# BaratiLab/GAMD

Measured on AMD Instinct MI355X. Metric: atom-steps/sec (force eval + integrate), 10k-atom LJ box, higher is better.
Workload: dtype f32; 1 GPU; C2: 10 000-atom LJ box, rho*=0.5, L=92.29 A, cutoff 3.0 sigma=10.2 A, fp32, 4 conv layers x 128, random-init weights (seed 0), 1 box per GPU; n_atoms=10000, boxes=1, launch=single process

## Files before the change

gamd_amd/csrc/conv_edge.hip:

```cpp
#include "gamd_common.h"
#include "gamd_internal.h"

#include <cstdlib>

namespace {

constexpr int conv_lds_floats(bool l0, bool fold = false) { return 2 * GAMD_WFRAG_FLOATS + 3 * 128 + (fold ? 256 : 0); }

template <bool F2, typename Post, typename Mid, typename Tail>
__device__ __forceinline__ void gemm128_post(const f32x4* W, int lane, const f32x16 (&X)[4], f32x16 (&acc)[4], Post post, Mid mid, Tail tail) {
#pragma unroll
    for (int tp = 0; tp < 4; ++tp) {
        if (tp == 1) mid();
#pragma unroll
        for (int t = 0; t < 4; ++t) {
#pragma unroll
            for (int q = 0; q < 4; ++q) {
                const f32x4 w = W[((tp * 4 + t) * 4 + q) * 64 + lane];
#pragma unroll
                for (int j = 0; j < 4; ++j) {
                    const float x = X[t][q * 4 + j];
                    acc[tp] = F2 ? mfma32(x, w[j], acc[tp]) : mfma32(w[j], x, acc[tp]);
                }
                if (tp > 0) post(tp - 1, t * 4 + q);
            }
        }
        tail(tp);
    }
#pragma unroll
    for (int g = 0; g < 16; ++g) post(3, g);
}
template <bool F2, typename Post, typename Mid>
__device__ __forceinline__ void gemm128_post(const f32x4* W, int lane, const f32x16 (&X)[4], f32x16 (&acc)[4], Post post, Mid mid) {
    gemm128_post<F2>(W, lane, X, acc, post, mid, [](int) {});
}

template <int N>
__device__ __forceinline__ void phase_barrier() {
    asm volatile("s_waitcnt vmcnt(%0) lgkmcnt(0)" ::"n"(N) : "memory");
    __builtin_amdgcn_s_barrier();
}

__device__ __forceinline__ void load_e_tile(const float* __restrict__ e_frag, int tile, int lane, f32x16 (&X)[4]) {
    const f32x4* ef = (const f32x4*)e_frag + (size_t)tile * 16 * 64;
#pragma unroll
    for (int t = 0; t < 4; ++t)
#pragma unroll
        for (int q = 0; q < 4; ++q) {
            const f32x4 v = gamd_load_stream(&ef[(t * 4 + q) * 64 + lane]);
#pragma unroll
            for (int j = 0; j < 4; ++j) X[t][q * 4 + j] = v[j];
        }
}

template <bool TIME, bool L0, bool FOLD = false>
__global__ void __launch_bounds__(512, 2) k_conv_edge(ConvEdgeArgs a) {
    if (a.devflags[DEVFLAG_FROZEN]) return;
    extern __shared__ __attribute__((aligned(16))) float lds[];
    float* buf0 = lds + (L0 ? 3 * 128 + (FOLD ? 256 : 0) : 0);
    float* buf1 = buf0 + GAMD_WFRAG_FLOATS;
    float* vb1 = L0 ? lds : buf1 + GAMD_WFRAG_FLOATS;
    float* vb3 = vb1 + 128;
    float* vb4 = vb3 + 128;
    float* vSD0 = vb4;
    float* vax = vb4 + 128;

    const int tid = threadIdx.x, lane = tid & 63, slot = lane & 31, half = lane >> 5;
    const int wave = __builtin_amdgcn_readfirstlane(tid >> 6);
    const unsigned lane16 = (unsigned)lane * 16u;
    int E = a.counters[CNT_E];
    if ((long long)E > a.e_cap) E = (int)a.e_cap;
    const int n_tiles = (E + GAMD_TILE - 1) / GAMD_TILE;
    const int n_units = (n_tiles + 3) / 4;
    int first, end, step;
    gamd_xcd_range(n_units, blockIdx.x, gridDim.x, first, end, step);
    if (first >= end) return;
    const int n_iter = ((end - first + step - 1) / step + 1) / 2;
    const int wsub = wave & 3, whalf = wave >> 2;
    const bool early = whalf == 0;
    auto tile_of = [&](int it) {
        const int u = first + (2 * it + whalf) * step;
        return (it < n_iter && u < end) ? u * 4 + wsub : n_tiles;
    };
    auto stage = [&](const float* gw, float* buf) { gamd_stage_weight_raw_contig<8>(gw, buf, wave, lane16); };

    long long tacc[16];
#pragma unroll
    for (int i = 0; i < 16; ++i) tacc[i] = 0;
    long long tprev = 0;
#define TMARK(i) do { if (TIME) { const long long tn__ = (long long)__builtin_readcyclecounter(); tacc[i] += tn__ - tprev; tprev = tn__; } } while (0)

    float vax_t = 0.f;
    if (FOLD && tid < 256) vax_t = a.w1p[GAMD_WFRAG_FLOATS + tid];
    if (tid < 128) {
        vb1[tid] = a.b1[tid]; vb3[tid] = a.b3[tid];
        if (L0) vSD0[tid] = a.S[tid] + a.D[tid];
        else vb4[tid] = a.b4[tid];
    }
    if (FOLD && tid < 256) vax[tid] = vax_t;
    stage(a.w1p, buf0);

    f32x16 RA[4], RB[4], RC[4];
    float rs = 0.f;
    float wxr[4] = {0.f, 0.f, 0.f, 0.f};
    auto fold_head = [&]() {
        if constexpr (FOLD) {
#pragma unroll
            for (int tp = 0; tp < 4; ++tp) wxr[tp] = vax[tp * 64 + lane];
            asm volatile("" : "+v"(wxr[0]), "+v"(wxr[1]), "+v"(wxr[2]), "+v"(wxr[3]));
        }
    };
    auto fold_tail = [&](int tp) { if constexpr (FOLD) RB[tp] = mfma32(wxr[tp], rs, RB[tp]); };
    auto init_b4 = [&]() {
#pragma unroll
        for (int tp = 0; tp < 4; ++tp) {
            const float b = vb4[32 * tp + slot];
#pragma unroll
            for (int r = 0; r < 16; ++r) RC[tp][r] = b;
        }
    };

    int tile = tile_of(0);
    bool active = tile < n_tiles;
    int src = 0, dst = 0;
    {
        const int x = tile * GAMD_TILE + gamd_pi(slot);
        if (active && x < E) {
            src = GAMD_CHK_RANGE(a.sticky, a.col[x], 0, a.zero_row, GAMD_CHK_CONV_SRC);
            if (!L0) dst = GAMD_CHK_RANGE(a.sticky, a.erow[x], 0, a.zero_row, GAMD_CHK_CONV_DST);
        } else { src = a.zero_row; dst = a.zero_row; }
        if (FOLD && active) rs = a.e_rstd[(size_t)tile * 64 + lane];
        if (active) load_e_tile(a.e_frag, tile, lane, RA);
    }
    asm volatile("" ::"v"(src), "v"(dst));
    asm volatile("s_waitcnt vmcnt(0)" ::: "memory");
    __syncthreads();
    if (TIME) tprev = (long long)__builtin_readcyclecounter();
    unsigned pend_ends = 0;
    int pend_p = 0;

    auto gather_S = [&]() { load_row_chain(a.S + (size_t)src * GAMD_H, half, RA); };
    auto gather_hn = [&]() {
        const unsigned soff = (unsigned)src << 9;
        const unsigned idx0 = 16u * (unsigned)half;
        const unsigned slot16 = 16u * (unsigned)slot;
#pragma unroll
        for (int r4 = 0; r4 < 4; ++r4) {
            unsigned o0, o1, o2, o3;
            asm volatile("ds_bpermute_b32 %0, %4, %5 offset:%6\n\tds_bpermute_b32 %1, %4, %5 offset:%7\n\t"
                         "ds_bpermute_b32 %2, %4, %5 offset:%8\n\tds_bpermute_b32 %3, %4, %5 offset:%9\n\ts_waitcnt lgkmcnt(0)"
                         : "=&v"(o0), "=&v"(o1), "=&v"(o2), "=&v"(o3)
                         : "v"(idx0), "v"(soff), "n"(4 * (0 + 8 * r4)), "n"(4 * (1 + 8 * r4)), "n"(4 * (2 + 8 * r4)), "n"(4 * (3 + 8 * r4)));
            const unsigned o[4] = {o0, o1, o2, o3};
#pragma unroll
            for (int k = 0; k < 4; ++k) {
                const f32x4 hv = *(const f32x4*)((const char*)a.hn + (o[k] + slot16));
#pragma unroll
                for (int tp = 0; tp < 4; ++tp) RA[r4][k * 4 + tp] = hv[tp];
            }
        }
    };

    auto early_barrier = [&](bool gathered) { if (gathered) phase_barrier<16>(); else phase_barrier<0>(); };
    auto early_barrier_e = [&](bool gathered) { if (gathered) phase_barrier<FOLD ? 17 : 16>(); else phase_barrier<0>(); };
    auto piece_stores = [&]() {
        while (__any(pend_ends != 0)) {
            if (pend_ends != 0) {
                const int r = __builtin_ctz(pend_ends);
                pend_ends &= pend_ends - 1;
                f32x4 pv;
#pragma unroll
                for (int tp = 0; tp < 4; ++tp) {
                    float v = RC[tp][0];
#pragma unroll
                    for (int k = 1; k < 16; ++k) v = (r == k) ? RC[tp][k] : v;
                    pv[tp] = v;
                }
                *(f32x4*)(a.partial + (size_t)pend_p * GAMD_H + 4 * slot) = pv;
                ++pend_p;
            }
        }
    };
#define FENCE() __builtin_amdgcn_sched_barrier(0)

    if constexpr (L0) {
    for (int it = 0; it < n_iter; ++it) {
        const int x0 = tile * GAMD_TILE + 16 * half;
        int nvalid = E - x0;
        nvalid = !active ? 0 : (nvalid >= 16 ? 16 : (nvalid <= 0 ? 0 : nvalid));
        const int tile_n = tile_of(it + 1);
// ... 199 lines not shown
```

gamd_amd/csrc/edge_encode.hip:

```cpp
#include "gamd_common.h"
#include "gamd_internal.h"

namespace {

constexpr int ENC_W1_FLOATS = 4 * 6 * 64 * 4;
constexpr int ENC_LDS_FLOATS = ENC_W1_FLOATS + 2 * GAMD_WFRAG_FLOATS + 5 * 128 + 64;
constexpr int ENC_R_FLOATS = 10 * 1024;

__device__ __forceinline__ constexpr int enc_r_block(int tp, int t) { return (tp == 0 ? 0 : tp == 1 ? 4 : tp == 2 ? 7 : 9) + (t - tp); }

template <typename WPtr, typename BPtr>
__device__ __forceinline__ void gemm128_upper_sq(WPtr W, BPtr b, int lane, int half, const f32x16 (&X)[4], float (&vt)[4]) {
#pragma unroll
    for (int tp = 0; tp < 4; ++tp) {
        f32x16 acc;
#pragma unroll
        for (int q = 0; q < 4; ++q) {
            const f32x4 v = *reinterpret_cast<const f32x4*>(&b[32 * tp + 8 * q + 4 * half]);
#pragma unroll
            for (int j = 0; j < 4; ++j) acc[q * 4 + j] = v[j];
        }
#pragma unroll
        for (int t = tp; t < 4; ++t)
#pragma unroll
            for (int q = 0; q < 4; ++q) {
                const f32x4 w = W[(enc_r_block(tp, t) * 4 + q) * 64 + lane];
#pragma unroll
                for (int j = 0; j < 4; ++j) acc = mfma32(w[j], X[t][q * 4 + j], acc);
            }
        vt[tp] = 0.f;
#pragma unroll
        for (int r = 0; r < 16; ++r) vt[tp] = fmaf(acc[r], acc[r], vt[tp]);
    }
}

template <int NFEAT, typename CPtr>
__device__ __forceinline__ void edge_features(const EncArgs& a, CPtr cen, int src, int dst, const float4& ps, const float4& pd,
                                              int half, float (&F)[24]) {
#pragma clang fp contract(off)
    const BoxDims B = gamd_edge_box(a, dst);
    const float rx = gamd_min_image_wrapped(ps.x - pd.x, B.bx, B.hx);
    const float ry = gamd_min_image_wrapped(ps.y - pd.y, B.by, B.hy);
    const float rz = gamd_min_image_wrapped(ps.z - pd.z, B.bz, B.hz);
    const float nrm = sqrtf((rx * rx + ry * ry) + rz * rz);
    const float den = nrm + 1e-8f;
    const float d = (nrm - a.length_mean) / a.length_std;
    F[0] = half ? ry / den : rx / den;
    F[1] = half ? d : rz / den;
    if (a.rbf.uniform) {
        gamd_rbf_chains(d, half, a.gamma * -1.4426950408889634f, a.rbf, F);
    } else {
#pragma unroll
        for (int s = 2; s < 22; ++s) {
            const float radial = d - cen[2 * (s - 2) + half];
            F[s] = __builtin_amdgcn_exp2f((a.gamma * -1.4426950408889634f) * (radial * radial));
        }
    }
    F[22] = 0.f; F[23] = 0.f;
    if (NFEAT == 45) {
        float flag = 0.f;
        if (a.bond_nbr) {
            const int io = a.perm[dst], jo = a.perm[src];
            const int4 nb = *reinterpret_cast<const int4*>(a.bond_nbr + 4 * (size_t)io);
            flag = (nb.x == jo || nb.y == jo || nb.z == jo || nb.w == jo) ? 1.f : 0.f;
        }
        F[22] = half ? 0.f : flag;
    }
}


__device__ __forceinline__ void gelu_block(const f32x16 (&acc)[4], f32x16 (&X)[4], const GeluCoef& k) {
    __builtin_amdgcn_s_setprio(1);
#pragma unroll
    for (int t = 0; t < 4; ++t)
#pragma unroll
        for (int r = 0; r < 16; r += 2) {
            const gelu_f2 y = gelu_pair(gelu_f2{acc[t][r], acc[t][r + 1]}, k);
            X[t][r] = y[0]; X[t][r + 1] = y[1];
        }
    __builtin_amdgcn_s_setprio(0);
}

template <int NFEAT, bool FOLD = false>
__global__ void __launch_bounds__(512, 2) k_edge_encode(EncArgs a) {
    if (a.devflags[DEVFLAG_FROZEN]) return;
    extern __shared__ __attribute__((aligned(16))) float lds[];
    float* w1 = lds;
    float* w2 = w1 + ENC_W1_FLOATS;
    float* w3 = w2 + GAMD_WFRAG_FLOATS;
    float* vb1 = w3 + GAMD_WFRAG_FLOATS;
    float* vb2 = vb1 + 128;
    float* vb3 = vb2 + 128;
    float* vg = vb3 + 128;
    float* vbeta = vg + 128;
    float* cen = vbeta + 128;

    const int tid = threadIdx.x;
    const GeluCoef gk = gelu_coef();
    for (int i = tid; i < ENC_W1_FLOATS / 4; i += 512) ((f32x4*)w1)[i] = ((const f32x4*)a.w1p)[i];
    for (int i = tid; i < GAMD_WFRAG_FLOATS / 4; i += 512) {
        ((f32x4*)w2)[i] = ((const f32x4*)a.w2p)[i];
        if (!FOLD || i < ENC_R_FLOATS / 4) ((f32x4*)w3)[i] = ((const f32x4*)a.w3p)[i];
    }
    if (tid < 128) {
        vb1[tid] = a.b1[tid]; vb2[tid] = a.b2[tid]; vb3[tid] = a.b3[tid];
        if (!FOLD) { vg[tid] = a.ln_g[tid]; vbeta[tid] = a.ln_b[tid]; }
    }
    if (tid < 40) cen[tid] = a.centers[tid];
    __syncthreads();

    const int lane = tid & 63, wave = tid >> 6, slot = lane & 31, half = lane >> 5;
    long long E = a.counters[CNT_E];
    if (E > a.e_cap) E = a.e_cap;
    const int n_tiles = (int)((E + GAMD_TILE - 1) / GAMD_TILE);
    const int n_units = (n_tiles + 3) / 4;
    int first, end, step;
    gamd_xcd_range(n_units, blockIdx.x, gridDim.x, first, end, step);
    const int n_iter = first < end ? ((end - first + step - 1) / step + 1) / 2 : 0;
    auto tile_of = [&](int it) {
        const int u = first + (2 * it + (wave >> 2)) * step;
        return (it < n_iter && u < end) ? u * 4 + (wave & 3) : n_tiles;
    };

    constexpr int KSTEPS = (NFEAT + 1) / 2;

    int E32 = (int)E;
    auto fetch_idx = [&](int tile, int& src, int& dst) -> bool {
        const int x = tile * GAMD_TILE + gamd_pi(slot);
        const bool ok = tile < n_tiles && x < E32;
        const int xc = ok ? x : 0;
        src = GAMD_CHK_RANGE(a.sticky, a.col[xc], 0, a.zero_row, GAMD_CHK_ENC_SRC); dst = GAMD_CHK_RANGE(a.sticky, a.erow[xc], 0, a.zero_row, GAMD_CHK_ENC_DST);
        return ok;
    };
    int src_c, dst_c;
    {
        const bool ok = fetch_idx(tile_of(0), src_c, dst_c);
        src_c = ok ? src_c : 0; dst_c = ok ? dst_c : 0;
    }
    float4 ps = a.pos_s[src_c], pd = a.pos_s[dst_c];

    for (int it = 0; it < n_iter; ++it) {
        const int tile = tile_of(it);
        int src_n, dst_n;
        const bool ok_n = fetch_idx(tile_of(it + 1), src_n, dst_n);
        if (tile >= n_tiles) { asm volatile("" ::"v"(src_n), "v"(dst_n)); continue; }
        const long long x = (long long)tile * GAMD_TILE + gamd_pi(slot);
        const bool valid = x < E;
        const int src = src_c, dst = dst_c;
        float F[24];
        __builtin_amdgcn_s_setprio(1);
        if constexpr (FOLD) edge_features<NFEAT>(a, a.centers, src, dst, ps, pd, half, F);
        else edge_features<NFEAT>(a, cen, src, dst, ps, pd, half, F);
        asm volatile("" : "+v"(F[0]), "+v"(F[23]));
        __builtin_amdgcn_s_setprio(0);
        if (a.feat_dbg && valid) {
#pragma unroll
            for (int s = 0; s < 24; ++s) a.feat_dbg[x * 48 + 2 * s + half] = F[s];
        }

        f32x16 acc[4], X[4];
        load_bias_chain(vb1, half, acc);
#pragma unroll
        for (int tp = 0; tp < 4; ++tp) {
#pragma unroll
            for (int g = 0; g < 6; ++g) {
                if (4 * g >= KSTEPS) break;
                const f32x4 w = ((const f32x4*)w1)[(tp * 6 + g) * 64 + lane];
#pragma unroll
                for (int j = 0; j < 4; ++j)
                    if (4 * g + j < KSTEPS) acc[tp] = mfma32(w[j], F[4 * g + j], acc[tp]);
            }
        }
        gelu_block(acc, X, gk);
        if constexpr (FOLD) {
#pragma unroll
            for (int t = 0; t < 4; ++t) asm volatile("" : "+v"(X[t]));
        }
        load_bias_chain(vb2, half, acc);
        gemm128<false>((const f32x4*)w2, lane, X, acc);
        gelu_block(acc, X, gk);
        src_c = ok_n ? src_n : 0; dst_c = ok_n ? dst_n : 0;
        ps = a.pos_s[src_c]; pd = a.pos_s[dst_c];
        if constexpr (FOLD) {
#pragma unroll
            for (int t = 0; t < 4; ++t) asm volatile("" : "+v"(X[t]));
            float vt[4];
            gemm128_upper_sq((const f32x4*)w3, vb3, lane, half, X, vt);
            const float var = gamd_xhalf_sum((vt[0] + vt[1]) + (vt[2] + vt[3])) * a.ln_inv_width;
            const float rstd = 1.0f / sqrtf(var + 1e-5f);
#pragma unroll
            for (int t = 0; t < 4; ++t)
#pragma unroll
                for (int r = 0; r < 16; ++r) acc[t][r] = X[t][r] * rstd;
// ... 172 lines not shown
```

gamd_amd/csrc/gamd_common.h:

```cpp
#pragma once
#include <hip/hip_runtime.h>
#include <stdint.h>

typedef float f32x16 __attribute__((ext_vector_type(16)));
typedef float f32x4 __attribute__((ext_vector_type(4)));

#define GAMD_H 128
#define GAMD_TILE 32
#define GAMD_CHUNK 16
#define GAMD_WFRAG_FLOATS (GAMD_H * GAMD_H)

__device__ __forceinline__ int gamd_pi(int rho) {
    return 16 * ((rho >> 2) & 1) + (rho & 3) + 4 * (rho >> 3);
}

__device__ __forceinline__ f32x16 mfma32(float a, float b, f32x16 c) {
    return __builtin_amdgcn_mfma_f32_32x32x2f32(a, b, c, 0, 0, 0);
}

template <bool F2, typename WPtr>
__device__ __forceinline__ void gemm128_tile(WPtr W, int lane, const f32x16 (&X)[4], f32x16& acc, int tp) {
#pragma unroll
    for (int t = 0; t < 4; ++t) {
#pragma unroll
// ... 51 lines not shown
    gelu_f2 d;
    asm("v_pk_fma_f32 %0, %1, %2, %3" : "=v"(d) : "v"(a), "v"(b), "v"(c));
    return d;
}
__device__ __forceinline__ gelu_f2 gelu_pair(gelu_f2 x, const GeluCoef& k) {
    const gelu_f2 a = {__builtin_amdgcn_fmed3f(fabsf(x[0]), 0.0f, 6.0f), __builtin_amdgcn_fmed3f(fabsf(x[1]), 0.0f, 6.0f)};
    gelu_f2 q = pk_fma(k.q[6], a, k.q[5]);
    q = pk_fma(q, a, k.q[4]);
    q = pk_fma(q, a, k.q[3]);
    q = pk_fma(q, a, k.q[2]);
    q = pk_fma(q, a, k.q[1]);
    q = pk_fma(q, a, k.q[0]);
    const gelu_f2 e = {__builtin_amdgcn_exp2f(q[0]), __builtin_amdgcn_exp2f(q[1])};
    const gelu_f2 relu = {x[0] - __builtin_amdgcn_fmed3f(x[0], -3.0e38f, 0.0f), x[1] - __builtin_amdgcn_fmed3f(x[1], -3.0e38f, 0.0f)};
    gelu_f2 r = {__builtin_fmaf(-a[0], e[0], relu[0]), __builtin_fmaf(-a[1], e[1], relu[1])};
    return r;
}

struct RbfGrid { int uniform; float c0, delta, A, B, C; };
__device__ __forceinline__ void gamd_rbf_chains(float d, int half, float gexp, const RbfGrid& g, float (&F)[24]) {
#pragma clang fp contract(off)
    const float s = 2.0f * g.delta;
    const float dh = d - (g.c0 + (half ? g.delta : 0.0f));
#pragma unroll
    for (int c = 0; c < 4; ++c) {
        const float u0 = dh - (float)(5 * c) * s;
        float v = __builtin_amdgcn_exp2f(gexp * (u0 * u0));
        float rho = __builtin_amdgcn_exp2f(fmaf(g.A, u0, g.B));
        F[2 + 5 * c] = v;
#pragma unroll
        for (int j = 1; j < 5; ++j) {
            v *= rho;
            F[2 + 5 * c + j] = v;
            if (j < 4) rho *= g.C;
        }
    }
}

__device__ __forceinline__ float gamd_remainder(float a, float b) {
    float m = fmodf(a, b);
    if (m != 0.0f && ((b < 0.0f) != (m < 0.0f))) m += b;
    return m;
}

__device__ __forceinline__ float gamd_min_image_wrapped(float d, float L, float halfL) {
    float t = d + halfL;
    if (t < 0.0f) t += L;
    else if (t >= L) t -= L;
    return t - halfL;
}

__device__ __forceinline__ f32x4 gamd_load_stream(const f32x4* p) { return __builtin_nontemporal_load(p); }

__device__ __forceinline__ float gamd_msg_acc(float hn, float e_emb, float prev) { return __builtin_fmaf(hn, e_emb, prev); }

#define GAMD_L0_PAD (-0x1p100f)
__device__ __forceinline__ float gamd_l0_acc(float pre, float prev) {
    const float e = __builtin_amdgcn_exp2f(pre * -1.4426950408889634f);
    return __builtin_fmaf(pre, __builtin_amdgcn_rcpf(1.0f + e), prev);
}

__host__ __device__ __forceinline__ int gamd_tab16_pos(int f) {
    return 16 * (2 * (f >> 5) + ((f >> 4) & 1)) + 8 * ((f >> 2) & 1) + 4 * ((f >> 3) & 1) + (f & 3);
}

template <typename BPtr>
__device__ __forceinline__ void load_bias_chain(BPtr b, int half, f32x16 (&acc)[4]) {
#pragma unroll
    for (int t = 0; t < 4; ++t)
#pragma unroll
        for (int q = 0; q < 4; ++q) {
            const f32x4 v = *reinterpret_cast<const f32x4*>(&b[32 * t + 8 * q + 4 * half]);
#pragma unroll
            for (int j = 0; j < 4; ++j) acc[t][q * 4 + j] = v[j];
        }
}

__device__ __forceinline__ void load_row_chain(const float* __restrict__ row, int half, f32x16 (&X)[4]) {
#pragma unroll
    for (int t = 0; t < 4; ++t)
#pragma unroll
        for (int q = 0; q < 4; ++q) {
            const f32x4 v = *reinterpret_cast<const f32x4*>(row + 32 * t + 8 * q + 4 * half);
#pragma unroll
            for (int j = 0; j < 4; ++j) X[t][q * 4 + j] = v[j];
        }
}

__device__ __forceinline__ void store_row_chain(float* __restrict__ row, int half, const f32x16 (&X)[4]) {
#pragma unroll
    for (int t = 0; t < 4; ++t)
#pragma unroll
        for (int q = 0; q < 4; ++q) {
            f32x4 v;
#pragma unroll
            for (int j = 0; j < 4; ++j) v[j] = X[t][q * 4 + j];
            *reinterpret_cast<f32x4*>(row + 32 * t + 8 * q + 4 * half) = v;
        }
}

__device__ __forceinline__ float gamd_xhalf_sum(float v) {
    return v + __shfl_xor(v, 32, 64);
}

template <typename GPtr>
__device__ __forceinline__ void layernorm_chain(f32x16 (&X)[4], GPtr gamma, GPtr beta, int half, float eps) {
// ... 20 lines not shown
            const f32x4 g = *reinterpret_cast<const f32x4*>(&gamma[32 * t + 8 * q + 4 * half]);
            const f32x4 b = *reinterpret_cast<const f32x4*>(&beta[32 * t + 8 * q + 4 * half]);
#pragma unroll
            for (int j = 0; j < 4; ++j) X[t][q * 4 + j] = (X[t][q * 4 + j] - mean) * rstd * g[j] + b[j];
        }
}

template <int NW = 8>
__device__ __forceinline__ void gamd_stage_weight(const float* __restrict__ gw, float* ldsbuf, int wave, unsigned lane16) {
    asm volatile("" : "+v"(lane16));
#pragma unroll
    for (int k = 0; k < 64 / NW; ++k) {
        const int chunk = k * NW + wave;
        const char* base = reinterpret_cast<const char*>(gw) + chunk * 1024;
        __builtin_amdgcn_global_load_lds(
            (const __attribute__((address_space(1))) void*)(base + lane16),
            (__attribute__((address_space(3))) void*)(ldsbuf + chunk * 256), 16, 0, 0);
    }
}

#pragma clang diagnostic push
#pragma clang diagnostic ignored "-Winline-asm"

template <int NW = 8>
__device__ __forceinline__ void gamd_stage_weight_raw(const float* __restrict__ gw, float* ldsbuf, int wave, unsigned lane16) {
    const unsigned lds0 = (unsigned)(size_t)(__attribute__((address_space(3))) float*)ldsbuf;
#pragma unroll
    for (int k = 0; k < 64 / NW; ++k) {
        const int chunk = k * NW + wave;
        asm volatile("s_mov_b32 m0, %2\n\ts_nop 0\n\tglobal_load_lds_dwordx4 %0, %1"
                     ::"v"(lane16), "s"(reinterpret_cast<const char*>(gw) + chunk * 1024), "s"(lds0 + chunk * 1024u)
                     : "memory", "m0");
    }
}

template <int NW = 8>
__device__ __forceinline__ void gamd_stage_weight_raw_contig(const float* __restrict__ gw, float* ldsbuf, int wave, unsigned lane16) {
    static_assert((64 / NW) % 4 == 0, "whole groups of four KiB-sized copies per wave");
    int woff = wave * (64 / NW) * 1024;
    asm volatile("" : "+s"(woff));
    const char* g0 = reinterpret_cast<const char*>(gw) + woff;
    const unsigned l0 = (unsigned)(size_t)(__attribute__((address_space(3))) float*)ldsbuf + (unsigned)woff;
#pragma unroll
    for (int h = 0; h < 64 / NW / 4; ++h)
        asm volatile("s_mov_b32 m0, %2\n\ts_nop 0\n\t"
                     "global_load_lds_dwordx4 %0, %1\n\t"
                     "global_load_lds_dwordx4 %0, %1 offset:1024\n\t"
                     "global_load_lds_dwordx4 %0, %1 offset:2048\n\t"
                     "global_load_lds_dwordx4 %0, %1 offset:3072"
                     ::"v"(lane16), "s"(g0 + h * 4096), "s"(l0 + h * 4096u)
                     : "memory", "m0");
}

#pragma clang diagnostic pop

struct WQuarter { f32x4 w[16]; };

__device__ __forceinline__ void load_wquarter(const float* __restrict__ Wp, int quarter, int lane, WQuarter& o) {
    const f32x4* W = reinterpret_cast<const f32x4*>(Wp) + (size_t)quarter * 16 * 64 + lane;
#pragma unroll
    for (int i = 0; i < 16; ++i) o.w[i] = W[i * 64];
}

template <bool F2 = false>
__device__ __forceinline__ void gemm_quarter(const WQuarter& wq, const f32x16 (&X)[4], f32x16& acc) {
#pragma unroll
    for (int t = 0; t < 4; ++t)
#pragma unroll
        for (int q = 0; q < 4; ++q)
#pragma unroll
            for (int j = 0; j < 4; ++j)
                acc = F2 ? mfma32(X[t][q * 4 + j], wq.w[t * 4 + q][j], acc) : mfma32(wq.w[t * 4 + q][j], X[t][q * 4 + j], acc);
}

__device__ __forceinline__ f32x16 load_slice(const float* __restrict__ row, int quarter, int half) {
    f32x16 v;
#pragma unroll
    for (int q = 0; q < 4; ++q) {
        const f32x4 x = *reinterpret_cast<const f32x4*>(row + 32 * quarter + 8 * q + 4 * half);
#pragma unroll
        for (int j = 0; j < 4; ++j) v[q * 4 + j] = x[j];
    }
    return v;
}

__device__ __forceinline__ void store_slice(float* __restrict__ row, int quarter, int half, const f32x16& v) {
#pragma unroll
    for (int q = 0; q < 4; ++q) {
        f32x4 x;
#pragma unroll
        for (int j = 0; j < 4; ++j) x[j] = v[q * 4 + j];
        *reinterpret_cast<f32x4*>(row + 32 * quarter + 8 * q + 4 * half) = x;
    }
}

template <int NB, int XLDW>
__device__ __forceinline__ void exchange_blocks(float* xbuf, int quarter, int slot, int half, const f32x16 (&mine)[NB],
                                                f32x16 (&X)[NB][4]) {
    __syncthreads();
#pragma unroll
    for (int b = 0; b < NB; ++b) store_slice(xbuf + slot * XLDW + 128 * b, quarter, half, mine[b]);
    __syncthreads();
#pragma unroll
    for (int b = 0; b < NB; ++b) load_row_chain(xbuf + slot * XLDW + 128 * b, half, X[b]);
}

// ... 44 lines not shown
```

gamd_amd/csrc/node.hip:

```cpp
#include "gamd_common.h"
#include "gamd_internal.h"

namespace {

typedef _Float16 nf16x8 __attribute__((ext_vector_type(8)));
typedef _Float16 nf16x2 __attribute__((ext_vector_type(2)));
typedef float nf32x2 __attribute__((ext_vector_type(2)));

constexpr int NT = 16;
constexpr int XLD = 136;

__device__ __forceinline__ f32x4 mfma16(float a, float b, f32x4 c) {
    return __builtin_amdgcn_mfma_f32_16x16x4f32(a, b, c, 0, 0, 0);
}

struct WHalf { f32x4 w[8]; };
__device__ __forceinline__ void load_whalf(const float* __restrict__ Wp, int w, int lane, int half, WHalf& h) {
    const f32x4* W = reinterpret_cast<const f32x4*>(Wp) + (size_t)w * 16 * 64 + lane;
#pragma unroll
    for (int o = 0; o < 2; ++o)
#pragma unroll
        for (int b = 0; b < 4; ++b) h.w[o * 4 + b] = W[(o * 8 + 4 * half + b) * 64];
}

// ... 46 lines not shown
    __builtin_amdgcn_sched_barrier(0);
    cur = wn;
    if (NEXT) {
        asm volatile("" ::: "memory");
        load_whalf(next, w, lane, 0, wn);
        asm volatile("" ::: "memory");
    }
    if constexpr (F16) gemm16_half_f16(cur, 1, XB, acc); else gemm16_half(cur, 1, XB, acc);
    __builtin_amdgcn_sched_barrier(0);
}

__device__ __forceinline__ void load16(const float* __restrict__ row, int w, int g, f32x4 (&v)[2]) {
    v[0] = *reinterpret_cast<const f32x4*>(row + 32 * w + 4 * g);
    v[1] = *reinterpret_cast<const f32x4*>(row + 32 * w + 16 + 4 * g);
}
__device__ __forceinline__ void store16(float* __restrict__ row, int w, int g, const f32x4 (&v)[2]) {
    *reinterpret_cast<f32x4*>(row + 32 * w + 4 * g) = v[0];
    *reinterpret_cast<f32x4*>(row + 32 * w + 16 + 4 * g) = v[1];
}

__device__ __forceinline__ void exchange16(float* xbuf, int w, int a, int g, const f32x4 (&mine)[2], f32x4 (&XB)[8]) {
    __syncthreads();
    store16(xbuf + a * XLD, w, g, mine);
    __syncthreads();
#pragma unroll
    for (int blk = 0; blk < 8; ++blk) XB[blk] = *reinterpret_cast<const f32x4*>(xbuf + a * XLD + 16 * blk + 4 * g);
}

typedef _Float16 nf16x4 __attribute__((ext_vector_type(4)));
__device__ __forceinline__ nf16x4 cvt16x4(const f32x4& v) {
    const nf16x2 lo = __builtin_convertvector(nf32x2{v[0], v[1]}, nf16x2), hi = __builtin_convertvector(nf32x2{v[2], v[3]}, nf16x2);
    return nf16x4{lo[0], lo[1], hi[0], hi[1]};
}
__device__ __forceinline__ void store16_h(_Float16* __restrict__ row, int w, int g, const f32x4 (&v)[2]) {
    *reinterpret_cast<nf16x4*>(row + 32 * w + 4 * g) = cvt16x4(v[0]);
    *reinterpret_cast<nf16x4*>(row + 32 * w + 16 + 4 * g) = cvt16x4(v[1]);
}
__device__ __forceinline__ void store16_tab(_Float16* __restrict__ row, int w, int g, const f32x4 (&v)[2]) {
    *reinterpret_cast<nf16x4*>(row + 32 * w + 8 * (g & 1) + 4 * (g >> 1)) = cvt16x4(v[0]);
    *reinterpret_cast<nf16x4*>(row + 32 * w + 16 + 8 * (g & 1) + 4 * (g >> 1)) = cvt16x4(v[1]);
}

__device__ __forceinline__ float group_sum(float v) {
    v += __shfl_xor(v, 16, 64);
    return v + __shfl_xor(v, 32, 64);
}

template <bool F16>
__global__ void __launch_bounds__(256, 3) k_node(NodeArgs a) {
    __shared__ __attribute__((aligned(16))) float xbuf[NT * XLD];
    __shared__ float obuf[4][NT][3];
    __shared__ float red[2][4][NT];

    if (a.counters[CNT_OVERFLOW] || a.devflags[DEVFLAG_FROZEN]) return;
    if (a.mode == 0 && a.l0_gate && a.counters[CNT_REBUILD] == 0) return;

    const int lane = threadIdx.x & 63, la = lane & 15, g = lane >> 4;
    const int w = __builtin_amdgcn_readfirstlane(threadIdx.x >> 6);
    const int atom_raw = blockIdx.x * NT + la;
    const bool valid = atom_raw < a.n;
    const int atom = valid ? atom_raw : a.n - 1;
    const size_t row = (size_t)atom * GAMD_H;

#ifdef GAMD_PROFILING
    long long tm[16] = {0, 0, 0, 0, 0, 0, 0, 0, 0, 0, 0, 0, 0, 0, 0, 0};
#define NMARK(I) do { if (a.tdbg) tm[I] = (long long)__builtin_readcyclecounter(); } while (0)
#else
#define NMARK(I) do { } while (0)
#endif
    NMARK(0);
    f32x4 XB[8];
    XSplit XS;
#define GEMM16(NEXT, W, NXT) do { if constexpr (F16) gemm16<NEXT, true>(W, NXT, wn, XS, mine, w, lane); \
                                  else gemm16<NEXT, false>(W, NXT, wn, XB, mine, w, lane); } while (0)
#define SPLIT16() do { if constexpr (F16) split16(XB, XS); } while (0)
    f32x4 mine[2];
    WHalf wn;

    if (a.mode == 0) {
        if (a.node_emb) {
            load16(a.node_emb, w, g, mine);
        } else {
            const float f = a.pos_s[atom].w;
            f32x4 ww[2];
            load16(a.enc_w, w, g, ww);
            load16(a.enc_b, w, g, mine);
#pragma unroll
            for (int o = 0; o < 2; ++o)
#pragma unroll
                for (int r = 0; r < 4; ++r) mine[o][r] = f * ww[o][r] + mine[o][r];
        }
        if (valid) store16(a.h_out + row, w, g, mine);
        load_whalf(a.pre.wsp, w, lane, 0, wn);
    } else {
        const int rp0 = a.row_ptr[atom], dg = a.deg[atom];
        const int na_incl = a.na_excl[atom] + ((dg > 0 && (rp0 % GAMD_CHUNK) != 0) ? 1 : 0);
        const int p0 = rp0 / GAMD_CHUNK + na_incl;
        const int np = dg > 0 ? ((rp0 + dg - 1) / GAMD_CHUNK - rp0 / GAMD_CHUNK + 1) : 0;
        (void)GAMD_CHK_RANGE(a.sticky, (long long)p0 + np, 0, a.piece_cap, GAMD_CHK_NODE_PIECES);
        float n_real = 0.f;
        if (a.post.c0) {
            float n_pad = 0.f;
            if (a.col) {
#pragma unroll
                for (int k = 0; k < 4; ++k) {
                    const int j = g + 4 * k;
                    if (j < dg && a.col[rp0 + dg - 1 - j] == a.n) n_pad += 1.f;
                }
                n_pad = group_sum(n_pad);
            }
            n_real = (float)dg - n_pad;
        }
        mine[0] = f32x4{0.f, 0.f, 0.f, 0.f};
        mine[1] = mine[0];
        f32x4 p_in[2], h_res[2];
        load16(a.P_in + row, w, g, p_in);
        for (int k0 = 0; __any(k0 < np); k0 += 8) {
            f32x4 pc[8][2];
#pragma unroll
            for (int k = 0; k < 8; ++k) {
                const int kk = (k0 + k < np) ? k0 + k : (np > 0 ? np - 1 : 0);
                load16(a.partial + (size_t)(np > 0 ? p0 + kk : 0) * GAMD_H, w, g, pc[k]);
            }
#pragma unroll
            for (int k = 0; k < 8; ++k)
                if (k0 + k < np) { mine[0] += pc[k][0]; mine[1] += pc[k][1]; }
        }
        NMARK(1);
        asm volatile("" ::: "memory");
        load_whalf(a.post.wpep, w, lane, 0, wn);
        exchange16(xbuf, w, la, g, mine, XB);
        SPLIT16();
        NMARK(2);
        mine[0] = p_in[0]; mine[1] = p_in[1];
        GEMM16(true, a.post.wpep, a.post.wphip);
        if (a.post.c0) {
            f32x4 c[2];
            load16(a.post.c0, w, g, c);
#pragma unroll
            for (int o = 0; o < 2; ++o)
#pragma unroll
                for (int r = 0; r < 4; ++r) mine[o][r] = fmaf(n_real, c[o][r], mine[o][r]);
        }
        NMARK(3);
#pragma unroll
        for (int o = 0; o < 2; ++o)
#pragma unroll
            for (int r = 0; r < 4; ++r) mine[o][r] = gamd_silu_hw(mine[o][r]);
        exchange16(xbuf, w, la, g, mine, XB);
        SPLIT16();
        NMARK(4);
        load16(a.post.bphi, w, g, mine);
        load16(a.h_in + row, w, g, h_res);
        GEMM16(true, a.post.wphip, a.mode != 2 ? a.pre.wsp : a.dec_w1p);
        mine[0] += h_res[0]; mine[1] += h_res[1];
        if (valid) store16(a.h_out + row, w, g, mine);
        NMARK(5);
    }

    if (a.mode != 2) {
        float mean = 0.f, rstd = 1.0f;
        if (!a.norm_bn) {
            float ps = 0.f;
#pragma unroll
            for (int o = 0; o < 2; ++o)
#pragma unroll
                for (int r = 0; r < 4; ++r) ps += mine[o][r];
            ps = group_sum(ps);
            if (g == 0) red[0][w][la] = ps;
// ... 111 lines not shown
```

Before: 3.403 million atom-steps/s.

## Overlap kernel prologue loads with device-flag and edge-count checks

The edge-conv, edge-encode and node kernels now issue the frozen/overflow/edge-count word loads through vector loads and read them later. Edge indices, biases, the first edge tile and the weight staging are issued speculatively before those values arrive, so the prologue memory latency overlaps instead of serialising behind the flag checks. A new tile-map header assigns each block a fixed first unit that needs no edge count, which makes the early speculative index loads possible, and weight staging in edge-encode switches to direct global-to-LDS copies. The cost is wasted speculative loads when the kernel exits early, plus added complexity in the tile scheduling.

```diff
diff --git a/gamd_amd/csrc/conv_edge.hip b/gamd_amd/csrc/conv_edge.hip
--- a/gamd_amd/csrc/conv_edge.hip
+++ b/gamd_amd/csrc/conv_edge.hip
@@ -1,5 +1,6 @@
 #include "gamd_common.h"
 #include "gamd_internal.h"
+#include "gamd_tile_map.h"
 
 #include <cstdlib>
 
@@ -55,7 +56,10 @@
 
 template <bool TIME, bool L0, bool FOLD = false>
 __global__ void __launch_bounds__(512, 2) k_conv_edge(ConvEdgeArgs a) {
-    if (a.devflags[DEVFLAG_FROZEN]) return;
+    const long long t_entry = TIME ? (long long)__builtin_readcyclecounter() : 0;
+    asm volatile("" ::"s"(a.devflags), "s"(a.counters), "s"(a.col), "s"(a.erow), "s"(a.e_frag), "s"(a.e_rstd), "s"(a.e_cap), "s"(a.w1p),
+                 "s"(a.b1), "s"(a.b3), "s"(a.b4), "s"(a.S), "s"(a.D), "s"(gridDim.x));
+    const int frozen_v = gamd_head_word_issue(a.devflags + DEVFLAG_FROZEN), E_v = gamd_head_word_issue(a.counters + CNT_E);
     extern __shared__ __attribute__((aligned(16))) float lds[];
     float* buf0 = lds + (L0 ? 3 * 128 + (FOLD ? 256 : 0) : 0);
     float* buf1 = buf0 + GAMD_WFRAG_FLOATS;
@@ -68,21 +72,41 @@
     const int tid = threadIdx.x, lane = tid & 63, slot = lane & 31, half = lane >> 5;
     const int wave = __builtin_amdgcn_readfirstlane(tid >> 6);
     const unsigned lane16 = (unsigned)lane * 16u;
-    int E = a.counters[CNT_E];
+    const int wsub = wave & 3, whalf = wave >> 2;
+    const bool early = whalf == 0;
+    auto stage = [&](const float* gw, float* buf) { gamd_stage_weight_raw_contig<8>(gw, buf, wave, lane16); };
+
+    f32x16 RA[4], RB[4], RC[4];
+    float rs = 0.f;
+    const int tile0 = gamd_tile_map_unit0(blockIdx.x, gridDim.x, whalf) * 4 + wsub;
+    const bool cap0 = (long long)tile0 * GAMD_TILE < a.e_cap;
+    int src_raw, dst_raw = 0;
+    {
+        const long long x = (long long)tile0 * GAMD_TILE + gamd_pi(slot);
+        const int xc = x < a.e_cap ? (int)x : 0;
+        src_raw = a.col[xc];
+        if (!L0) dst_raw = a.erow[xc];
+    }
+    if (FOLD && cap0 && early) rs = a.e_rstd[(size_t)tile0 * 64 + lane];
+    if (cap0 && early) load_e_tile(a.e_frag, tile0, lane, RA);
+    float vax_t = 0.f, vb1_t = 0.f, vb3_t = 0.f, vb4_t = 0.f, vd0_t = 0.f;
+    if (FOLD && tid < 256) vax_t = a.w1p[GAMD_WFRAG_FLOATS + tid];
+    if (tid < 128) {
+        vb1_t = a.b1[tid]; vb3_t = a.b3[tid];
+        if (L0) { vb4_t = a.S[tid]; vd0_t = a.D[tid]; }
+        else vb4_t = a.b4[tid];
+    }
+    stage(a.w1p, buf0);
+    asm volatile("" ::: "memory");
+    if (gamd_head_word(frozen_v)) { asm volatile("s_waitcnt vmcnt(0)" ::: "memory"); return; }
+    int E = gamd_head_word(E_v);
     if ((long long)E > a.e_cap) E = (int)a.e_cap;
     const int n_tiles = (E + GAMD_TILE - 1) / GAMD_TILE;
     const int n_units = (n_tiles + 3) / 4;
-    int first, end, step;
-    gamd_xcd_range(n_units, blockIdx.x, gridDim.x, first, end, step);
-    if (first >= end) return;
-    const int n_iter = ((end - first + step - 1) / step + 1) / 2;
-    const int wsub = wave & 3, whalf = wave >> 2;
-    const bool early = whalf == 0;
-    auto tile_of = [&](int it) {
-        const int u = first + (2 * it + whalf) * step;
-        return (it < n_iter && u < end) ? u * 4 + wsub : n_tiles;
-    };
-    auto stage = [&](const float* gw, float* buf) { gamd_stage_weight_raw_contig<8>(gw, buf, wave, lane16); };
+    const GamdTileMap tmap = gamd_tile_map(n_units, blockIdx.x, gridDim.x);
+    if (tmap.n_iter == 0) { asm volatile("s_waitcnt vmcnt(0)" ::: "memory"); return; }
+    const int n_iter = tmap.n_iter;
+    auto tile_of = [&](int it) { return gamd_tile_map_tile_later(tmap, it, whalf, wsub, n_tiles); };
 
     long long tacc[16];
 #pragma unroll
@@ -90,18 +114,6 @@
     long long tprev = 0;
 #define TMARK(i) do { if (TIME) { const long long tn__ = (long long)__builtin_readcyclecounter(); tacc[i] += tn__ - tprev; tprev = tn__; } } while (0)
 
-    float vax_t = 0.f;
-    if (FOLD && tid < 256) vax_t = a.w1p[GAMD_WFRAG_FLOATS + tid];
-    if (tid < 128) {
-        vb1[tid] = a.b1[tid]; vb3[tid] = a.b3[tid];
-        if (L0) vSD0[tid] = a.S[tid] + a.D[tid];
-        else vb4[tid] = a.b4[tid];
-    }
-    if (FOLD && tid < 256) vax[tid] = vax_t;
-    stage(a.w1p, buf0);
-
-    f32x16 RA[4], RB[4], RC[4];
-    float rs = 0.f;
     float wxr[4] = {0.f, 0.f, 0.f, 0.f};
     auto fold_head = [&]() {
         if constexpr (FOLD) {
@@ -120,22 +132,30 @@
         }
     };
 
-    int tile = tile_of(0);
+    int tile = gamd_tile_map_tile(tmap, 0, whalf, wsub, n_tiles);
     bool active = tile < n_tiles;
-    int src = 0, dst = 0;
+    int src = a.zero_row, dst = L0 ? 0 : a.zero_row;
     {
         const int x = tile * GAMD_TILE + gamd_pi(slot);
         if (active && x < E) {
-            src = GAMD_CHK_RANGE(a.sticky, a.col[x], 0, a.zero_row, GAMD_CHK_CONV_SRC);
-            if (!L0) dst = GAMD_CHK_RANGE(a.sticky, a.erow[x], 0, a.zero_row, GAMD_CHK_CONV_DST);
-        } else { src = a.zero_row; dst = a.zero_row; }
-        if (FOLD && active) rs = a.e_rstd[(size_t)tile * 64 + lane];
-        if (active) load_e_tile(a.e_frag, tile, lane, RA);
+            src = GAMD_CHK_RANGE(a.sticky, src_raw, 0, a.zero_row, GAMD_CHK_CONV_SRC);
+            if (!L0) dst = GAMD_CHK_RANGE(a.sticky, dst_raw, 0, a.zero_row, GAMD_CHK_CONV_DST);
+        }
     }
     asm volatile("" ::"v"(src), "v"(dst));
+    if (tid < 128) {
+        vb1[tid] = vb1_t; vb3[tid] = vb3_t;
+        if (L0) vSD0[tid] = vb4_t + vd0_t;
+        else vb4[tid] = vb4_t;
+    }
+    if (FOLD && tid < 256) vax[tid] = vax_t;
     asm volatile("s_waitcnt vmcnt(0)" ::: "memory");
     __syncthreads();
-    if (TIME) tprev = (long long)__builtin_readcyclecounter();
+    if (!early && active) {
+        if (FOLD) rs = a.e_rstd[(size_t)tile * 64 + lane];
+        load_e_tile(a.e_frag, tile, lane, RA);
+    }
+    if (TIME) { tprev = (long long)__builtin_readcyclecounter(); tacc[14] = tprev - t_entry; }
     unsigned pend_ends = 0;
     int pend_p = 0;
 
diff --git a/gamd_amd/csrc/edge_encode.hip b/gamd_amd/csrc/edge_encode.hip
--- a/gamd_amd/csrc/edge_encode.hip
+++ b/gamd_amd/csrc/edge_encode.hip
@@ -1,5 +1,6 @@
 #include "gamd_common.h"
 #include "gamd_internal.h"
+#include "gamd_tile_map.h"
 
 namespace {
 
@@ -83,7 +84,24 @@
 
 template <int NFEAT, bool FOLD = false>
 __global__ void __launch_bounds__(512, 2) k_edge_encode(EncArgs a) {
-    if (a.devflags[DEVFLAG_FROZEN]) return;
+    asm volatile("" ::"s"(a.devflags), "s"(a.counters), "s"(a.col), "s"(a.erow), "s"(a.e_cap), "s"(a.pos_s), "s"(a.w1p), "s"(a.w2p), "s"(a.w3p),
+                 "s"(gridDim.x));
+    const int frozen_v = gamd_head_word_issue(a.devflags + DEVFLAG_FROZEN), E_v = gamd_head_word_issue(a.counters + CNT_E);
+    int src_raw, dst_raw;
+    {
+        const int wave0 = __builtin_amdgcn_readfirstlane(threadIdx.x >> 6);
+        const long long x = (long long)(gamd_tile_map_unit0(blockIdx.x, gridDim.x, wave0 >> 2) * 4 + (wave0 & 3)) * GAMD_TILE + gamd_pi(threadIdx.x & 31);
+        const int xc = x < a.e_cap ? (int)x : 0;
+        src_raw = a.col[xc]; dst_raw = a.erow[xc];
+    }
+    float vb_t[5] = {0.f, 0.f, 0.f, 0.f, 0.f}, cen_t = 0.f;
+    if (threadIdx.x < 128) {
+        vb_t[0] = a.b1[threadIdx.x]; vb_t[1] = a.b2[threadIdx.x]; vb_t[2] = a.b3[threadIdx.x];
+        if (!FOLD) { vb_t[3] = a.ln_g[threadIdx.x]; vb_t[4] = a.ln_b[threadIdx.x]; }
+    }
+    if (!FOLD && threadIdx.x < 40) cen_t = a.centers[threadIdx.x];
+    asm volatile("" ::: "memory");
+    if (gamd_head_word(frozen_v)) return;
     extern __shared__ __attribute__((aligned(16))) float lds[];
     float* w1 = lds;
     float* w2 = w1 + ENC_W1_FLOATS;
@@ -97,34 +115,45 @@
 
     const int tid = threadIdx.x;
     const GeluCoef gk = gelu_coef();
-    for (int i = tid; i < ENC_W1_FLOATS / 4; i += 512) ((f32x4*)w1)[i] = ((const f32x4*)a.w1p)[i];
-    for (int i = tid; i < GAMD_WFRAG_FLOATS / 4; i += 512) {
-        ((f32x4*)w2)[i] = ((const f32x4*)a.w2p)[i];
-        if (!FOLD || i < ENC_R_FLOATS / 4) ((f32x4*)w3)[i] = ((const f32x4*)a.w3p)[i];
-    }
-    if (tid < 128) {
-        vb1[tid] = a.b1[tid]; vb2[tid] = a.b2[tid]; vb3[tid] = a.b3[tid];
-        if (!FOLD) { vg[tid] = a.ln_g[tid]; vbeta[tid] = a.ln_b[tid]; }
-    }
-    if (tid < 40) cen[tid] = a.centers[tid];
-    __syncthreads();
-
     const int lane = tid & 63, wave = tid >> 6, slot = lane & 31, half = lane >> 5;
-    long long E = a.counters[CNT_E];
+    long long E = gamd_head_word(E_v);
     if (E > a.e_cap) E = a.e_cap;
     const int n_tiles = (int)((E + GAMD_TILE - 1) / GAMD_TILE);
     const int n_units = (n_tiles + 3) / 4;
-    int first, end, step;
-    gamd_xcd_range(n_units, blockIdx.x, gridDim.x, first, end, step);
-    const int n_iter = first < end ? ((end - first + step - 1) / step + 1) / 2 : 0;
-    auto tile_of = [&](int it) {
-        const int u = first + (2 * it + (wave >> 2)) * step;
-        return (it < n_iter && u < end) ? u * 4 + (wave & 3) : n_tiles;
-    };
+    const GamdTileMap tmap = gamd_tile_map(n_units, blockIdx.x, gridDim.x);
+    const int n_iter = tmap.n_iter;
+    if (n_iter == 0) return;
+    const int E32 = (int)E;
+    int src_c = 0, dst_c = 0;
+    {
+        const int tile = gamd_tile_map_tile(tmap, 0, wave >> 2, wave & 3, n_tiles);
+        if (tile < n_tiles && tile * GAMD_TILE + gamd_pi(slot) < E32) {
+            src_c = GAMD_CHK_RANGE(a.sticky, src_raw, 0, a.zero_row, GAMD_CHK_ENC_SRC); dst_c = GAMD_CHK_RANGE(a.sticky, dst_raw, 0, a.zero_row, GAMD_CHK_ENC_DST);
+        }
+    }
+    float4 ps = a.pos_s[src_c], pd = a.pos_s[dst_c];
+    if (tid < 128) {
+        vb1[tid] = vb_t[0]; vb2[tid] = vb_t[1]; vb3[tid] = vb_t[2];
+        if (!FOLD) { vg[tid] = vb_t[3]; vbeta[tid] = vb_t[4]; }
+    }
+    if (!FOLD && tid < 40) cen[tid] = cen_t;
+    asm volatile("" ::: "memory");
+    constexpr int G1 = ENC_W1_FLOATS / 256 / 8, G2 = GAMD_WFRAG_FLOATS / 256 / 8, G3 = (FOLD ? ENC_R_FLOATS : GAMD_WFRAG_FLOATS) / 256 / 8;
+    static_assert(G1 * 8 * 256 == ENC_W1_FLOATS && G3 * 8 * 256 == (FOLD ? ENC_R_FLOATS : GAMD_WFRAG_FLOATS), "whole KiB-sized copies per wave");
+    {
+        const int wave_s = __builtin_amdgcn_readfirstlane(tid >> 6);
+        const unsigned lane16 = (unsigned)lane * 16u;
+        gamd_stage_raw_contig_chunks<G1>(a.w1p, w1, wave_s, lane16);
+        gamd_stage_raw_contig_chunks<G2>(a.w2p, w2, wave_s, lane16);
+        gamd_stage_raw_contig_chunks<G3>(a.w3p, w3, wave_s, lane16);
+    }
+    asm volatile("s_waitcnt vmcnt(0) lgkmcnt(0)" ::: "memory");
+    __builtin_amdgcn_s_barrier();
+
+    auto tile_of = [&](int it) { return gamd_tile_map_tile(tmap, it, wave >> 2, wave & 3, n_tiles); };
 
     constexpr int KSTEPS = (NFEAT + 1) / 2;
 
-    int E32 = (int)E;
     auto fetch_idx = [&](int tile, int& src, int& dst) -> bool {
         const int x = tile * GAMD_TILE + gamd_pi(slot);
         const bool ok = tile < n_tiles && x < E32;
@@ -132,13 +161,6 @@
         src = GAMD_CHK_RANGE(a.sticky, a.col[xc], 0, a.zero_row, GAMD_CHK_ENC_SRC); dst = GAMD_CHK_RANGE(a.sticky, a.erow[xc], 0, a.zero_row, GAMD_CHK_ENC_DST);
         return ok;
     };
-    int src_c, dst_c;
-    {
-        const bool ok = fetch_idx(tile_of(0), src_c, dst_c);
-        src_c = ok ? src_c : 0; dst_c = ok ? dst_c : 0;
-    }
-    float4 ps = a.pos_s[src_c], pd = a.pos_s[dst_c];
-
     for (int it = 0; it < n_iter; ++it) {
         const int tile = tile_of(it);
         int src_n, dst_n;
diff --git a/gamd_amd/csrc/gamd_common.h b/gamd_amd/csrc/gamd_common.h
--- a/gamd_amd/csrc/gamd_common.h
+++ b/gamd_amd/csrc/gamd_common.h
@@ -127,6 +127,13 @@
 
 __device__ __forceinline__ f32x4 gamd_load_stream(const f32x4* p) { return __builtin_nontemporal_load(p); }
 
+__device__ __forceinline__ int gamd_head_word_issue(const int* p) {
+    unsigned z = 0;
+    asm volatile("" : "+v"(z));
+    return p[z];
+}
+__device__ __forceinline__ int gamd_head_word(int v) { return __builtin_amdgcn_readfirstlane(v); }
+
 __device__ __forceinline__ float gamd_msg_acc(float hn, float e_emb, float prev) { return __builtin_fmaf(hn, e_emb, prev); }
 
 #define GAMD_L0_PAD (-0x1p100f)
@@ -253,6 +260,31 @@
                      : "memory", "m0");
 }
 
+template <int CNT>
+__device__ __forceinline__ void gamd_stage_raw_group(unsigned lane16, const char* g, unsigned l) {
+    static_assert(CNT >= 1 && CNT <= 4, "one base pair reaches four KiB-sized copies");
+    if constexpr (CNT == 4)
+        asm volatile("s_mov_b32 m0, %2\n\ts_nop 0\n\tglobal_load_lds_dwordx4 %0, %1\n\tglobal_load_lds_dwordx4 %0, %1 offset:1024\n\t"
+                     "global_load_lds_dwordx4 %0, %1 offset:2048\n\tglobal_load_lds_dwordx4 %0, %1 offset:3072" ::"v"(lane16), "s"(g), "s"(l) : "memory", "m0");
+    else if constexpr (CNT == 3)
+        asm volatile("s_mov_b32 m0, %2\n\ts_nop 0\n\tglobal_load_lds_dwordx4 %0, %1\n\tglobal_load_lds_dwordx4 %0, %1 offset:1024\n\t"
+                     "global_load_lds_dwordx4 %0, %1 offset:2048" ::"v"(lane16), "s"(g), "s"(l) : "memory", "m0");
+    else if constexpr (CNT == 2)
+        asm volatile("s_mov_b32 m0, %2\n\ts_nop 0\n\tglobal_load_lds_dwordx4 %0, %1\n\tglobal_load_lds_dwordx4 %0, %1 offset:1024" ::"v"(lane16), "s"(g), "s"(l) : "memory", "m0");
+    else
+        asm volatile("s_mov_b32 m0, %2\n\ts_nop 0\n\tglobal_load_lds_dwordx4 %0, %1" ::"v"(lane16), "s"(g), "s"(l) : "memory", "m0");
+}
+template <int NCHUNK>
+__device__ __forceinline__ void gamd_stage_raw_contig_chunks(const float* __restrict__ gw, float* ldsbuf, int wave, unsigned lane16) {
+    int woff = wave * NCHUNK * 1024;
+    asm volatile("" : "+s"(woff));
+    const char* g0 = reinterpret_cast<const char*>(gw) + woff;
+    const unsigned l0 = (unsigned)(size_t)(__attribute__((address_space(3))) float*)ldsbuf + (unsigned)woff;
+#pragma unroll
+    for (int h = 0; h < NCHUNK / 4; ++h) gamd_stage_raw_group<4>(lane16, g0 + h * 4096, l0 + h * 4096u);
+    if constexpr (NCHUNK % 4 != 0) gamd_stage_raw_group<NCHUNK % 4>(lane16, g0 + (NCHUNK / 4) * 4096, l0 + (NCHUNK / 4) * 4096u);
+}
+
 #pragma clang diagnostic pop
 
 struct WQuarter { f32x4 w[16]; };
diff --git a/gamd_amd/csrc/gamd_tile_map.h b/gamd_amd/csrc/gamd_tile_map.h
--- /dev/null
+++ b/gamd_amd/csrc/gamd_tile_map.h
@@ -0,0 +1,63 @@
+#pragma once
+
+#if defined(__HIPCC__) || defined(__CUDACC__)
+#define GAMD_TM_HD __host__ __device__ __forceinline__
+#else
+#define GAMD_TM_HD inline
+#endif
+
+struct GamdTileMap {
+    int n_units;
+    int first0;
+    int stride0;
+    int first;
+    int end;
+    int step;
+    int n_iter;
+};
+
+GAMD_TM_HD int gamd_tile_map_unit0(int block, int n_blocks, int whalf) { return block + whalf * n_blocks; }
+
+GAMD_TM_HD GamdTileMap gamd_tile_map(int n_units, int block, int n_blocks) {
+    GamdTileMap m;
+    m.n_units = n_units;
+    m.first0 = block;
+    m.stride0 = n_blocks;
+    const int base = 2 * n_blocks;
+    const int rest = n_units > base ? n_units - base : 0;
+    const int nx = 8;
+    if (n_blocks % nx != 0 || n_blocks < nx) {
+        m.first = base + block; m.end = base + rest; m.step = n_blocks;
+    } else {
+        const int x = block % nx, w = block / nx, per = n_blocks / nx;
+        const int q = rest / nx, rem = rest % nx;
+        const int lo = x * q + (x < rem ? x : rem);
+        const int cnt = q + (x < rem ? 1 : 0);
+        m.first = base + lo + w; m.end = base + lo + cnt; m.step = per;
+    }
+    const int later = m.first < m.end ? (m.end - m.first + m.step - 1) / m.step : 0;
+    m.n_iter = (block < n_units ? 1 : 0) + (later + 1) / 2;
+    return m;
+}
+
+GAMD_TM_HD int gamd_tile_map_unit_later(const GamdTileMap& m, int it, int whalf) {
+    const int u = m.first + (2 * (it - 1) + whalf) * m.step;
+    return (it < m.n_iter && u < m.end) ? u : -1;
+}
+
+GAMD_TM_HD int gamd_tile_map_unit(const GamdTileMap& m, int it, int whalf) {
+    if (it > 0) return gamd_tile_map_unit_later(m, it, whalf);
+    const int u = m.first0 + whalf * m.stride0;
+    return u < m.n_units ? u : -1;
+}
+
+GAMD_TM_HD int gamd_tile_map_tile_of_unit(int u, int wsub, int n_tiles) {
+    const int t = u * 4 + wsub;
+    return (u >= 0 && t < n_tiles) ? t : n_tiles;
+}
+GAMD_TM_HD int gamd_tile_map_tile(const GamdTileMap& m, int it, int whalf, int wsub, int n_tiles) {
+    return gamd_tile_map_tile_of_unit(gamd_tile_map_unit(m, it, whalf), wsub, n_tiles);
+}
+GAMD_TM_HD int gamd_tile_map_tile_later(const GamdTileMap& m, int it, int whalf, int wsub, int n_tiles) {
+    return gamd_tile_map_tile_of_unit(gamd_tile_map_unit_later(m, it, whalf), wsub, n_tiles);
+}
diff --git a/gamd_amd/csrc/node.hip b/gamd_amd/csrc/node.hip
--- a/gamd_amd/csrc/node.hip
+++ b/gamd_amd/csrc/node.hip
@@ -122,8 +122,9 @@
     __shared__ float obuf[4][NT][3];
     __shared__ float red[2][4][NT];
 
-    if (a.counters[CNT_OVERFLOW] || a.devflags[DEVFLAG_FROZEN]) return;
-    if (a.mode == 0 && a.l0_gate && a.counters[CNT_REBUILD] == 0) return;
+    asm volatile("" ::"s"(a.counters), "s"(a.devflags), "s"(a.row_ptr), "s"(a.deg), "s"(a.na_excl), "s"(a.P_in), "s"(a.n), "s"(a.mode), "s"(a.l0_gate));
+    const int overflow_v = gamd_head_word_issue(a.counters + CNT_OVERFLOW), frozen_v = gamd_head_word_issue(a.devflags + DEVFLAG_FROZEN);
+    const int rebuild_v = gamd_head_word_issue(a.counters + CNT_REBUILD);
 
     const int lane = threadIdx.x & 63, la = lane & 15, g = lane >> 4;
     const int w = __builtin_amdgcn_readfirstlane(threadIdx.x >> 6);
@@ -131,6 +132,15 @@
     const bool valid = atom_raw < a.n;
     const int atom = valid ? atom_raw : a.n - 1;
     const size_t row = (size_t)atom * GAMD_H;
+    int rp0 = 0, dg = 0, na_ex = 0;
+    f32x4 p_in[2] = {f32x4{0.f, 0.f, 0.f, 0.f}, f32x4{0.f, 0.f, 0.f, 0.f}};
+    if (a.mode != 0) {
+        rp0 = a.row_ptr[atom]; dg = a.deg[atom]; na_ex = a.na_excl[atom];
+        load16(a.P_in + row, w, g, p_in);
+    }
+    asm volatile("" ::: "memory");
+    if (gamd_head_word(overflow_v) || gamd_head_word(frozen_v)) return;
+    if (a.mode == 0 && a.l0_gate && gamd_head_word(rebuild_v) == 0) return;
 
 #ifdef GAMD_PROFILING
     long long tm[16] = {0, 0, 0, 0, 0, 0, 0, 0, 0, 0, 0, 0, 0, 0, 0, 0};
@@ -163,8 +173,7 @@
         if (valid) store16(a.h_out + row, w, g, mine);
         load_whalf(a.pre.wsp, w, lane, 0, wn);
     } else {
-        const int rp0 = a.row_ptr[atom], dg = a.deg[atom];
-        const int na_incl = a.na_excl[atom] + ((dg > 0 && (rp0 % GAMD_CHUNK) != 0) ? 1 : 0);
+        const int na_incl = na_ex + ((dg > 0 && (rp0 % GAMD_CHUNK) != 0) ? 1 : 0);
         const int p0 = rp0 / GAMD_CHUNK + na_incl;
         const int np = dg > 0 ? ((rp0 + dg - 1) / GAMD_CHUNK - rp0 / GAMD_CHUNK + 1) : 0;
         (void)GAMD_CHK_RANGE(a.sticky, (long long)p0 + np, 0, a.piece_cap, GAMD_CHK_NODE_PIECES);
@@ -183,8 +192,7 @@
         }
         mine[0] = f32x4{0.f, 0.f, 0.f, 0.f};
         mine[1] = mine[0];
-        f32x4 p_in[2], h_res[2];
-        load16(a.P_in + row, w, g, p_in);
+        f32x4 h_res[2];
         for (int k0 = 0; __any(k0 < np); k0 += 8) {
             f32x4 pc[8][2];
 #pragma unroll
```

New measurement: 3.427 million atom-steps/s (median of 6 runs). No clear change (+0.7%).
